# wtsi-svi/ReadServer

Hardware: AMD Instinct MI355X
Metric: 31-mer backward-search queries/sec on popBWT, counted as (query x shard) backward searches/s (higher is better)
Workload: dtype u64

## Files before the change

readserver_amd/csrc/search_solo.h:

```cpp
#ifndef RSBWT_SEARCH_SOLO_H
#define RSBWT_SEARCH_SOLO_H

namespace rsb {

constexpr uint64_t WL_DEAD = 1ull << 63;
constexpr uint32_t SOLO_STAGED_RESULTS = 4u;
constexpr uint32_t SOLO_COUNT_UNSTAGED = 8u;
constexpr uint32_t RES_WAVE_LDS = 2048u;
constexpr uint32_t SOLO_RESULTS_LDS = WG_WAVES * RES_WAVE_LDS;
constexpr uint32_t RES_SLOT_BYTES = 8u;
constexpr uint32_t RES_STATE_BYTES = 8u;
constexpr uint32_t RES_BUFS = RES_WAVE_LDS / (8u * RES_SLOT_BYTES + RES_STATE_BYTES);
static_assert(RES_BUFS * (8u * RES_SLOT_BYTES + RES_STATE_BYTES) <= RES_WAVE_LDS, "a wave's buffers and their state fit its 2 KB");
static_assert(RES_WAVE_LDS == 2048u && RES_BUFS == 28u, "2 KB per wave: with the line slots a CU's 160 KB at four workgroups");
static_assert(RES_BUFS >= 9u && RES_BUFS <= 64u, "a lane per buffer claims; at most 9 groups begin among a pass's 64 draws");
constexpr uint32_t RES_WIDTH_BITS = 24u;
constexpr uint32_t RES_ESCAPED = (1u << RES_WIDTH_BITS) - 1u;

__device__ __forceinline__ void solo_lds_handoff() {
    __builtin_amdgcn_fence(__ATOMIC_RELEASE, "wavefront", "local");
    __builtin_amdgcn_wave_barrier();
    __builtin_amdgcn_fence(__ATOMIC_ACQUIRE, "wavefront", "local");
}

#ifndef RSB_WALK1MM_WGS_PER_CU
#define RSB_WALK1MM_WGS_PER_CU 3
#endif
template <bool COUNT_WORK, bool COUNTS_ONLY, bool LONGK, bool FUSED = false, bool WL = false, bool WALK = false>
__global__ void __launch_bounds__(64 * WG_WAVES, WALK ? RSB_WALK1MM_WGS_PER_CU : RSB_MIN_WGS_PER_CU)
search_solo_kernel(const shard_view *__restrict__ shards, uint32_t nshards, const uint64_t *__restrict__ packed,
                   const ulonglong2 *__restrict__ init, const uint8_t *__restrict__ valid,
                   unsigned long long *__restrict__ next_query,
                   size_t Q, uint32_t k, uint32_t wpq,
                   uint64_t *__restrict__ out_lower, uint64_t *__restrict__ out_upper,
                   unsigned long long *__restrict__ work,
                   ulonglong2 *__restrict__ trace, uint32_t trace_n, uint32_t qchunk, uint32_t pairs_arg,
                   const unsigned long long *__restrict__ wl_counts = nullptr, size_t wl_cap = 0, size_t wl_implicit = 0) {
    __shared__ uint4 s_stage[WG_WAVES][64 * SLOT_U4];
    extern __shared__ uint4 s_results[];
    const uint32_t lane = threadIdx.x & 63u;
    const uint32_t wave = threadIdx.x >> 6;
    uint4 *stage = s_stage[wave];
    const uint32_t stage_lds = __builtin_amdgcn_readfirstlane((uint32_t)(uintptr_t)(lds_void_ptr)stage);
    const uint32_t swz = lane & 7u;
    const uint32_t pairs = pairs_arg & 3u;
    constexpr bool CAN_STAGE = !COUNTS_ONLY && !WL && !WALK;
    const bool stage_out = CAN_STAGE && (pairs_arg & SOLO_STAGED_RESULTS) != 0u && pairs != 2u && Q < (1ull << 34);
    uint2 *results = reinterpret_cast<uint2 *>(s_results + wave * (RES_WAVE_LDS / 16u));
    uint32_t *res_state = reinterpret_cast<uint32_t *>(results + RES_BUFS * 8u);
    const bool count_unstaged = COUNT_WORK && (pairs_arg & SOLO_COUNT_UNSTAGED) != 0u;
    const lds_u32 *mine0 = reinterpret_cast<const lds_u32 *>(stage + (lane & 7u) * 64u + (lane >> 3) * SLOT_U4);
#define SOLO_MINE(d) (mine0 + (((((uint32_t)(d)) >> 2) ^ swz) << 2) + (((uint32_t)(d)) & 3u))

    unsigned long long w_steps = 0, w_occ = 0, w_lines = 0, w_hops = 0, w_ktab = 0, passes = 0;
    unsigned long long w_surv = 0, w_unstepped = 0;
    unsigned long long w_unstaged = 0;

    uint32_t sid = blockIdx.x % nshards;
    for (uint32_t visited = 0; visited < nshards; ++visited, sid = (sid + 1u == nshards) ? 0u : sid + 1u) {
        const shard_view *sv = shards + sid;
        const char *lines_bytes = reinterpret_cast<const char *>(sv->lines);
        const uint32_t S = sv->sp.S;
        const double inv = sv->sp.inv;
        const uint32_t nlines = (uint32_t)sv->nlines;
        const bool ktab = view_uses_ktab(*sv, k);
        const int j_table = ktab ? (int)(k - sv->ktab_depth) - 1 : (int)k - 2;
        const uint32_t w_table = j_table > 0 ? (uint32_t)j_table >> 5 : 0u;
        const ulonglong2 *init_s = WL ? init + (size_t)sid * wl_cap * 2u : init + (size_t)sid * Q;
        const size_t Qs = WALK ? Q : WL ? wl_implicit + (size_t)(wl_counts[(size_t)sid * WL_COUNT_STRIDE] < wl_cap ? wl_counts[(size_t)sid * WL_COUNT_STRIDE] : wl_cap) : Q;
        const uint32_t wl_tn = trace_n, wl_per = WL ? 3u * (k - trace_n) : 1u;
        const size_t walk_V = 3u * (size_t)k + 1u, walk_mv = Q * walk_V;
        ulonglong2 *walk_wl = WALK ? const_cast<ulonglong2 *>(init) + (size_t)sid * wl_cap * 2u : nullptr;
        unsigned long long *walk_count = WALK ? const_cast<unsigned long long *>(wl_counts) + (size_t)sid * WL_COUNT_STRIDE : nullptr;
        uint64_t *out_lo = WALK ? out_lower + (size_t)sid * walk_mv * 2u : out_lower + (size_t)sid * Q * (pairs ? 2u : 1u);
        uint64_t *out_up = (COUNTS_ONLY || pairs) ? nullptr : out_upper + (size_t)sid * Q;
        unsigned long long *pool = next_query + (size_t)sid * POOL_STRIDE;
        if (visited != 0u && __hip_atomic_load(pool, __ATOMIC_RELAXED, __HIP_MEMORY_SCOPE_AGENT) >= (unsigned long long)Qs) continue;
        ulonglong2 *trace_s = (trace && !WL) ? trace + (size_t)sid * Q * trace_n : nullptr;
        const uint64_t *wl_pre = (WL && trace) ? reinterpret_cast<const uint64_t *>(trace) + (size_t)sid * wl_implicit : nullptr;
        unsigned long long *hit_map = pairs == 2u ? reinterpret_cast<unsigned long long *>(out_upper) + (size_t)sid * hit_map_words(WALK ? walk_mv : Q) : nullptr;
        uint32_t ctab_lo, ctab_hi;
        {
            const uint64_t c1 = sv->C[1], c2 = sv->C[2], c3 = sv->C[3], c4 = sv->C[4];
            const uint32_t l3 = lane & 3u;
            const uint64_t cv = l3 == 0u ? c1 : l3 == 1u ? c2 : l3 == 2u ? c3 : c4;
            ctab_lo = (uint32_t)cv;
            ctab_hi = (uint32_t)(cv >> 32);
        }

        const uint64_t *__restrict__ ktab_p = sv->ktab;
        const uint32_t ktab_T = sv->ktab_depth, ktab_stride = sv->ktab_stride, ktab_fmt = sv->ktab_fmt;
        const uint64_t ix_n = sv->n;
        const uint64_t sc1 = sv->C[1], sc2 = sv->C[2], sc3 = sv->C[3], sc4 = sv->C[4];
        const uint64_t st1 = sv->total[1], st2 = sv->total[2], st3 = sv->total[3], st4 = sv->total[4];

        const uint32_t QCHUNK = qchunk;
        if (CAN_STAGE && stage_out && lane < RES_BUFS) {
            res_state[2u * lane] = ~0u;
            res_state[2u * lane + 1u] = 0u;
        }
        uint64_t pool_next = 0, pool_end = 0;
        bool drained = false;
        size_t q = 0;
        bool has_q = false;
        size_t nq = 0;
        bool has_n = false;
        ulonglong2 nrec = {0, 0};
        uint64_t nword = 0;
        uint32_t nstage = 0;
        bool nimp = false;
        int j = 0;
        uint64_t word = 0, lo = 0, hi = 0;
        uint32_t sub = 0;
        uint64_t occL = 0, cacc = 0;
        uint32_t cont = 0, cblk = 0, cdw = 0, co = 0, tries = 0, w = 0;
        uint64_t altL0 = 0, altL1 = 0, altL2 = 0, altU0 = 0, altU1 = 0, altU2 = 0;
        bool alt_ok = true;

        for (;;) {
            bool done = false;
            bool last_in = false;
            if (FUSED && !has_q && has_n && nstage == 2u) {
                const uint64_t e = nrec.x;
                const uint32_t width = (uint32_t)(e >> COUNT_BITS);
                if (nrec.y == 0ull) {
                    nrec.x = INIT_INVALID;
                } else if (width != KTAB_WIDE && (e & COUNT_MASK) + width <= ix_n) {
                    nrec.x = e & COUNT_MASK;
                    nrec.y = nrec.x + width - 1ull;
                } else {
                    const uint32_t bl = (uint32_t)((nword >> (2u * ((k - 1u) & 31u))) & 3u);
                    const uint64_t cb = bl == 0u ? sc1 : bl == 1u ? sc2 : bl == 2u ? sc3 : sc4;
                    const uint64_t tb = bl == 0u ? st1 : bl == 1u ? st2 : bl == 2u ? st3 : st4;
                    nrec.x = cb | INIT_FALLBACK;
                    nrec.y = cb + tb - 1ull;
                }
            }
            if (WL && !has_q && has_n && nstage == 2u) {
                has_q = true;
                has_n = false;
                sub = 0;
                cont = 0;
                word = nword;
                if (nimp) {
                    const uint32_t r_ = (uint32_t)(nrec.y >> 8) & 0xFFu, q_ = (uint32_t)(nrec.y >> 32);
                    const uint32_t pr = (r_ * 171u) >> 9;
                    q = (size_t)q_ * (3u * k + 1u) + 1u + 3u * (wl_tn + pr) + (r_ - 3u * pr);
                    const uint64_t e = nrec.x;
                    const uint32_t width = (uint32_t)(e >> COUNT_BITS);
                    bool tabulated = false;
                    if (width != KTAB_WIDE && (e & COUNT_MASK) + width <= ix_n) {
                        lo = e & COUNT_MASK;
                        hi = lo + width - 1ull;
                        j = (int)wl_tn - 1;
                        tabulated = true;
                    } else {
                        const uint32_t bl = (uint32_t)((nword >> (2u * ((k - 1u) & 31u))) & 3u);
                        const uint64_t cb = bl == 0u ? sc1 : bl == 1u ? sc2 : bl == 2u ? sc3 : sc4;
                        const uint64_t tb = bl == 0u ? st1 : bl == 1u ? st2 : bl == 2u ? st3 : st4;
                        lo = cb;
                        hi = cb + tb - 1ull;
                        j = (int)k - 2;
                    }
                    done = (nrec.y & 0xFFull) == 0ull || (tabulated && lo > hi) || j < 0;
                } else {
                    q = nq;
                    lo = nrec.x & COUNT_MASK;
                    hi = nrec.y;
                    j = (int)((nrec.x >> COUNT_BITS) & 0xFFFFull);
                    done = (nrec.x & WL_DEAD) != 0ull || lo > hi;
                }
                if (done) { lo = 1; hi = 0; }
            }
            if (!WL && !has_q && has_n && (!FUSED || nstage == 2u)) {
                has_q = true;
                has_n = false;
                q = nq;
                sub = 0;
                cont = 0;
                if (nrec.x & INIT_INVALID) {
                    lo = 1;
                    hi = 0;
                    j = -1;
                    done = true;
                } else if (nrec.x & INIT_EXPLICIT) {
                    lo = nrec.x & COUNT_MASK;
                    hi = nrec.y;
                    j = (int)((nrec.x >> COUNT_BITS) & 0xFFFFull) - ((nrec.x & INIT_VAR) ? 1 : 0);
                    word = nword;
                    done = j < 0 || ((nrec.x & INIT_NOCHECK) == 0ull && lo > hi);
                    if (LONGK) {
                        if (!done && ((uint32_t)j >> 5) != w_table) word = packed[q * wpq + ((uint32_t)j >> 5)];
                    }
                } else {
                    const bool fallback = !ktab || (nrec.x & INIT_FALLBACK) != 0ull;
                    lo = nrec.x & COUNT_MASK;
                    hi = nrec.y;
                    j = fallback ? (int)k - 2 : j_table;
                    word = nword;
                    if (COUNT_WORK && !fallback) w_ktab += 1;
                    done = (j < 0) || (!fallback && lo > hi);
                    if (LONGK) {
                        if (!done && ((uint32_t)j >> 5) != w_table) word = packed[q * wpq + ((uint32_t)j >> 5)];
                    }
                }
            }
            if (pool_next >= pool_end && !drained) {
                unsigned long long c = 0;
                if (lane == 0u) c = atomicAdd(pool, (unsigned long long)QCHUNK);
                c = ((unsigned long long)__builtin_amdgcn_readfirstlane((uint32_t)(c >> 32)) << 32) |
                    __builtin_amdgcn_readfirstlane((uint32_t)c);
                pool_next = c;
                pool_end = c + QCHUNK < Qs ? c + QCHUNK : Qs;
                if (c >= Qs) { drained = true; pool_next = pool_end = 0; }
            }
            bool got_n = false;
            {
                const uint64_t want_mask = __builtin_amdgcn_ballot_w64(!has_n);
                const uint32_t before = (uint32_t)__builtin_popcountll(want_mask & ((1ull << lane) - 1ull));
                const uint64_t mine = pool_next + before;
                if (!has_n && mine < pool_end) {
                    nq = (size_t)mine;
                    got_n = true;
                }
                const uint64_t taken = pool_next + (uint32_t)__builtin_popcountll(want_mask);
                const uint64_t r0 = pool_next;
                pool_next = taken < pool_end ? taken : pool_end;
                if (CAN_STAGE && stage_out && pool_next > r0) {
                    const uint64_t first = (r0 + 7ull) & ~7ull;
                    if (first < pool_next) {
                        const uint32_t ga = (uint32_t)(first >> 3), gb = (uint32_t)((pool_next - 1ull) >> 3) + 1u;
                        const uint32_t gam = ga % RES_BUFS;
                        if (lane < RES_BUFS) {
                            const uint32_t d = lane >= gam ? lane - gam : lane + RES_BUFS - gam;
                            const uint32_t g = ga + d;
                            if (g < gb && res_state[2u * lane + 1u] == 0u) {
                                const uint64_t q0 = (uint64_t)g << 3;
                                res_state[2u * lane] = g;
                                res_state[2u * lane + 1u] = (uint32_t)((q0 + 8ull < pool_end ? q0 + 8ull : pool_end) - q0);
                            }
                        }
                    }
                    solo_lds_handoff();
                }
            }
            if (__builtin_amdgcn_ballot_w64(has_q || got_n || ((FUSED || WL) && has_n)) == 0ull) {
                if (drained) break;
                continue;
            }
            ulonglong2 rec = {0, 0};
            uint64_t first_word = 0;
            const bool stage_b = (FUSED || WL) && has_n && nstage == 1u;
            uint64_t entry = 0;
            uint64_t wl_index = 0, vword = 0;
            bool imp = false;
            if (WL) {
                if (got_n) {
                    imp = nq < wl_implicit;
                    if (imp) {
                        const uint32_t i32 = (uint32_t)nq, q_ = i32 / wl_per, r_ = i32 - q_ * wl_per;
                        first_word = packed[q_];
                        rec.y = (uint64_t)valid[q_] | ((uint64_t)r_ << 8) | ((uint64_t)q_ << 32);
                    } else {
                        const size_t slot = nq - wl_implicit;
                        rec = init_s[2u * slot];
                        const ulonglong2 r2 = init_s[2u * slot + 1u];
                        wl_index = r2.x;
                        first_word = r2.y;
                    }
                }
                if (stage_b) {
                    const uint32_t r_ = (uint32_t)(nrec.y >> 8) & 0xFFu;
                    const uint32_t pr = (r_ * 171u) >> 9, d_ = r_ - 3u * pr, p_ = wl_tn + pr;
                    const uint32_t orig = (uint32_t)((nword >> (2u * p_)) & 3u);
                    const uint32_t alt = d_ < orig ? d_ : d_ + 1u;
                    vword = nword ^ ((uint64_t)(orig ^ alt) << (2u * p_));
                    const uint64_t code = (vword >> (2u * wl_tn)) & ((1ull << (2u * ktab_T)) - 1ull);
                    entry = wl_pre ? wl_pre[nq] : ktab_entry(ktab_p, ktab_fmt, ktab_T, ktab_stride, code);
                }
            } else if (FUSED) {
                if (got_n) {
                    rec.y = valid[nq];
                    first_word = packed[nq];
                }
                if (stage_b) {
                    const uint64_t code = (nword >> (2u * (k - ktab_T))) & ((1ull << (2u * ktab_T)) - 1ull);
                    entry = ktab_entry(ktab_p, ktab_fmt, ktab_T, ktab_stride, code);
                }
            } else if (got_n) {
                rec = init_s[nq];
                first_word = packed[nq * wpq + w_table];
            }
            const bool alive = has_q;
            const bool stepping = alive && !done;
            const bool fresh = stepping && cont == 0u;

            uint32_t b = 1, line = 0, o = 0;
            if (stepping) {
                if (LONGK) {
                    if (fresh && sub == 0u && (j & 31) == 31) word = packed[q * wpq + ((uint32_t)j >> 5)];
                }
                b = (uint32_t)((word >> (2u * ((uint32_t)j & 31u))) & 3u) + 1u;
            }
            bool no_fetch = false;
            if (fresh) {
                if (sub == 0u) {
                    if (WALK) {
                        alt_ok = true;
                        altL0 = altL1 = altL2 = altU0 = altU1 = altU2 = 0;
                    }
                    if (trace_s && (uint32_t)j < trace_n) trace_s[q * trace_n + (uint32_t)j] = make_ulonglong2(lo, hi);
                    if (lo == 0ull) {
                        occL = 0;
                        sub = 1u;
                    }
                }
                const uint64_t p = sub ? hi : lo - 1ull;
                if (p == ~0ull) {
                    no_fetch = true;
                } else {
                    uint32_t pin;
                    w = fast_window(p, S, inv, pin);
                    line = w + (w >> GROUP_SHIFT);
                    o = pin + 1u;
                    if (line >= nlines) line = 0;
                    if (COUNT_WORK) w_occ += 1;
                }
            }
            const bool looking = stepping && !no_fetch;
            const uint64_t pb = ((uint64_t)(uint32_t)__builtin_amdgcn_ds_bpermute((int)((b - 1u) << 2), (int)ctab_hi) << 32) |
                                (uint32_t)__builtin_amdgcn_ds_bpermute((int)((b - 1u) << 2), (int)ctab_lo);

            const uint32_t want = looking ? (cont ? cblk : line) : ~0u;
            if (COUNT_WORK && want != ~0u) {
                if (cont) w_hops += 1;
                else w_lines += 1;
            }
            glds_fetch(lines_bytes, want, lane, stage_lds);
            glds_wait();

            bool do_scan = false, own_line = false;
            uint64_t base = 0, cnt_b = 0;
            uint32_t dw = HDR_DWORDS, rem = 0, oe_here = 0;
            uint32_t s1 = 0, s2 = 0, s3 = 0, span = 0, hb = 0;
            const sym_tab stab = make_sym_tab(b);
            if (looking) {
                if (cont != KIND_CHUNK) {
                    const uint32_t oe = cont ? co : o;
                    const uint2 cw = *reinterpret_cast<const lds_u2 *>(SOLO_MINE(2u * (b - 1u)));
                    const uint4 h0 = *reinterpret_cast<const lds_u4 *>(SOLO_MINE(0));
                    const uint64_t cnt = ((uint64_t)(cw.y & 0xFFu) << 32) | cw.x;
                    const uint32_t m0 = h0.y >> 8, m1 = h0.w >> 8;
                    s1 = m0 & 0x3FFu;
                    s2 = (m0 >> 10) & 0x7FFu;
                    s3 = s2 + (m1 & 0x3FFu);
                    span = s3 + ((m1 >> 10) & 0x3FFu);
                    const uint32_t kind = (m1 >> 20) & 3u;
                    if (oe <= span) {
                        const uint32_t cq = (oe > s1 ? 1u : 0u) + (oe > s2 ? 1u : 0u) + (oe > s3 ? 1u : 0u);
                        const uint32_t start = cq == 0u ? 0u : cq == 1u ? s1 : cq == 2u ? s2 : s3;
                        const uint32_t hm = *SOLO_MINE(5u + 2u * ((b - 1u) >> 1)) >> 8;
                        hb = (hm >> (11u * ((b - 1u) & 1u))) & 0x7FFu;
                        const uint32_t qd = HDR_DWORDS + 6u * (cq & 2u);
                        const uint2 x0 = *reinterpret_cast<const lds_u2 *>(SOLO_MINE(qd));
                        const uint2 x1 = *reinterpret_cast<const lds_u2 *>(SOLO_MINE(qd + 2u));
                        const uint2 x2 = *reinterpret_cast<const lds_u2 *>(SOLO_MINE(qd + 4u));
                        const uint32_t e6[6] = {x0.x, x0.y, x1.x, x1.y, x2.x, x2.y};
                        const uint32_t m = matched24_tab(e6, stab);
                        base = cnt + (cq >= 2u ? hb : 0u) + ((cq & 1u) ? m : 0u);
                        dw = HDR_DWORDS + 6u * cq;
                        rem = oe - start;
                        do_scan = true;
                        own_line = true;
                        oe_here = oe;
                        cnt_b = cnt;
                    } else if (kind == KIND_FAR) {
                        cblk = *SOLO_MINE(LINE_DWORDS - 1u);
                        if (cblk >= nlines) cblk = 0;
                        cont = KIND_FAR;
                        co = oe - span;
                    } else if (kind == KIND_CHUNK && cont == 0u) {
                        const uint32_t m2 = *SOLO_MINE(5) >> 8, m3 = *SOLO_MINE(7) >> 8;
                        cacc = cnt;
                        cdw = 2u * (((m2 >> 22) & 3u) | (((m3 >> 22) & 3u) << 2));
                        cblk = (w >> GROUP_SHIFT) * (GROUP + 1u) + GROUP;
                        if (cblk >= nlines) cblk = 0;
                        cont = KIND_CHUNK;
                        co = oe - span;
                    } else {
                        base = cnt;
                        do_scan = true;
                    }
                } else {
                    const uint2 hd = *reinterpret_cast<const lds_u2 *>(SOLO_MINE(cdw));
                    const uint32_t hw = (b <= 2u) ? hd.x : hd.y;
                    const uint32_t tot = (hw >> (12u * ((b - 1u) & 1u))) & 0xFFFu;
                    base = cacc + tot;
                    dw = cdw + 2u;
                    rem = co;
                    do_scan = true;
                }
                if (!do_scan && ++tries > 72u) do_scan = true;
            }
            uint64_t occ = 0;
            {
                const uint2 y0 = *reinterpret_cast<const lds_u2 *>(SOLO_MINE(dw & 31u));
                const uint2 y1 = *reinterpret_cast<const lds_u2 *>(SOLO_MINE((dw + 2u) & 31u));
                const uint2 y2 = *reinterpret_cast<const lds_u2 *>(SOLO_MINE((dw + 4u) & 31u));
                const uint32_t r6[6] = {y0.x, y0.y, y1.x, y1.y, y2.x, y2.y};
                occ = base + rank24(r6, stab, b, rem);
#ifdef RSB_FAULT_INJECT_WILD_OCC
                if ((((uint32_t)q + (uint32_t)j) * 2654435761u >> 28) == 0u)
                    occ = (occ + (((uint64_t)q * 0x9E3779B97F4A7C15ull) >> (23u + (((uint32_t)q + (uint32_t)j) & 31u)))) & ((1ull << 41) - 1ull);
#endif
            }
            bool step_done = false;
            uint64_t occU = 0;
            bool second = false;
            uint32_t oh = 0;
            bool ev1 = false, ev1_is_L = false;
            if (WALK && do_scan && (uint32_t)j < trace_n) {
                if (own_line) {
                    ev1 = true;
                    ev1_is_L = sub == 0u;
                } else {
                    alt_ok = false;
                }
            }
            if (do_scan) {
                cont = 0;
                tries = 0;
                if (sub == 0u) {
                    occL = occ;
                    sub = 1u;
                    const uint64_t d = hi - (lo - 1ull);
                    if (own_line && d <= (uint64_t)(span - oe_here)) {
                        second = true;
                        oh = oe_here + (uint32_t)d;
                    }
                } else {
                    occU = occ;
                    step_done = true;
                }
            }
            {
                const uint32_t cq = (oh > s1 ? 1u : 0u) + (oh > s2 ? 1u : 0u) + (oh > s3 ? 1u : 0u);
                const uint32_t start = cq == 0u ? 0u : cq == 1u ? s1 : cq == 2u ? s2 : s3;
                const uint32_t qd = HDR_DWORDS + 6u * (cq & 2u);
                const uint2 x0 = *reinterpret_cast<const lds_u2 *>(SOLO_MINE(qd));
                const uint2 x1 = *reinterpret_cast<const lds_u2 *>(SOLO_MINE(qd + 2u));
                const uint2 x2 = *reinterpret_cast<const lds_u2 *>(SOLO_MINE(qd + 4u));
                const uint32_t e6[6] = {x0.x, x0.y, x1.x, x1.y, x2.x, x2.y};
                const uint32_t m = matched24_tab(e6, stab);
                const uint32_t dw2 = HDR_DWORDS + 6u * cq;
                const uint2 y0 = *reinterpret_cast<const lds_u2 *>(SOLO_MINE(dw2));
                const uint2 y1 = *reinterpret_cast<const lds_u2 *>(SOLO_MINE(dw2 + 2u));
                const uint2 y2 = *reinterpret_cast<const lds_u2 *>(SOLO_MINE(dw2 + 4u));
                const uint32_t r6[6] = {y0.x, y0.y, y1.x, y1.y, y2.x, y2.y};
                const uint32_t sc = rank24(r6, stab, b, second ? oh - start : 0u);
                if (second) {
                    occU = cnt_b + (cq >= 2u ? hb : 0u) + ((cq & 1u) ? m : 0u) + sc;
                    step_done = true;
                    if (COUNT_WORK) w_occ += 1;
                }
            }
            if (stepping && no_fetch) {
                occU = 0;
                step_done = true;
            }
            if (WALK) {
                const staged_line Lrow = {mine0, swz};
                const line_head hh = {s1, s2, s3, span, 0u};
#pragma unroll 1
                for (uint32_t ev = 0; ev < 2u; ++ev) {
                    const bool want = ev == 0u ? ev1 : (second && (uint32_t)j < trace_n);
                    if (__builtin_amdgcn_ballot_w64(want) == 0ull) continue;
                    uint64_t t3[3];
                    staged_occ_alts(Lrow, hh, want ? (ev == 0u ? oe_here : oh) : 1u, b - 1u, t3);
                    if (want) {
                        if (ev == 0u && ev1_is_L) { altL0 = t3[0]; altL1 = t3[1]; altL2 = t3[2]; }
                        else { altU0 = t3[0]; altU1 = t3[1]; altU2 = t3[2]; }
                    }
                }
                const bool emit = step_done && (uint32_t)j < trace_n;
                if (__builtin_amdgcn_ballot_w64(emit) != 0ull) {
                    const uint32_t orig = b - 1u;
                    uint64_t nlo[3], nhi[3], masks[3];
                    bool enq[3];
#pragma unroll
                    for (uint32_t d = 0; d < 3u; ++d) {
                        const uint32_t alt = d < orig ? d : d + 1u;
                        const uint64_t cb = ((uint64_t)(uint32_t)__builtin_amdgcn_ds_bpermute((int)(alt << 2), (int)ctab_hi) << 32) |
                                            (uint32_t)__builtin_amdgcn_ds_bpermute((int)(alt << 2), (int)ctab_lo);
                        nlo[d] = cb + (d == 0u ? altL0 : d == 1u ? altL1 : altL2);
                        nhi[d] = cb + (d == 0u ? altU0 : d == 1u ? altU1 : altU2) - 1ull;
                        const bool stepped_live = emit && alt_ok && nlo[d] <= nhi[d];
                        const bool final_hit = stepped_live && j == 0;
                        enq[d] = (stepped_live && j != 0) || (emit && !alt_ok);
                        if (final_hit) {
                            const size_t canon = q * walk_V + 1u + 3u * (uint32_t)j + d;
                            reinterpret_cast<ulonglong2 *>(out_lo)[canon] = make_ulonglong2(nlo[d], nhi[d]);
                            atomicOr(hit_map + (canon >> 6), 1ull << (canon & 63u));
                        }
                        masks[d] = __builtin_amdgcn_ballot_w64(enq[d]);
                        if (COUNT_WORK) {
                            w_surv += __builtin_popcountll(__builtin_amdgcn_ballot_w64((enq[d] && alt_ok) || final_hit));
                            w_unstepped += __builtin_popcountll(__builtin_amdgcn_ballot_w64(enq[d] && !alt_ok));
                        }
                    }
                    if (COUNT_WORK && emit) w_steps += 3;
                    const uint32_t n0 = (uint32_t)__builtin_popcountll(masks[0]), n1 = (uint32_t)__builtin_popcountll(masks[1]);
                    const uint32_t total = n0 + n1 + (uint32_t)__builtin_popcountll(masks[2]);
                    if (total != 0u) {
                        unsigned long long wbase = 0;
                        if (lane == 0u) wbase = atomicAdd(walk_count, (unsigned long long)total);
                        wbase = ((unsigned long long)(uint32_t)__builtin_amdgcn_readfirstlane((int)(uint32_t)(wbase >> 32)) << 32) |
                                (uint32_t)__builtin_amdgcn_readfirstlane((int)(uint32_t)wbase);
                        const uint64_t lt = (1ull << lane) - 1ull;
#pragma unroll
                        for (uint32_t d = 0; d < 3u; ++d) {
                            if (!enq[d]) continue;
                            const size_t slot = (size_t)wbase + (d >= 1u ? n0 : 0u) + (d >= 2u ? n1 : 0u) + (size_t)__builtin_popcountll(masks[d] & lt);
                            if (slot >= wl_cap) continue;
                            const uint32_t alt = d < orig ? d : d + 1u;
                            const uint64_t vword = word ^ ((uint64_t)(orig ^ alt) << (2u * (uint32_t)j));
                            const uint64_t canon = (uint64_t)q * walk_V + 1ull + 3ull * (uint32_t)j + d;
                            if (!alt_ok) wl_store(walk_wl, slot, lo, (uint32_t)j, hi, canon, vword);
                            else wl_store(walk_wl, slot, nlo[d], (uint32_t)j - 1u, nhi[d], canon, vword);
                        }
                    }
                }
            }
            if (step_done) {
                if (COUNT_WORK) w_steps += 1;
                lo = pb + occL;
                hi = pb + occU - 1ull;
                --j;
                done = (lo > hi) || (j < 0);
                sub = 0;
            }
            if ((FUSED || WL) && stage_b) {
                nrec.x = entry;
                nstage = 2u;
                if (WL) nword = vword;
            }
            if (got_n) {
                nrec = rec;
                nword = first_word;
                has_n = true;
                nstage = (WL && !imp) ? 2u : 1u;
                nimp = imp;
                if (WL && !imp) nq = (size_t)wl_index;
            }
            if (CAN_STAGE && stage_out) solo_lds_handoff();
            if (alive && done) {
                if (trace_s) {
                    for (int jj = j < (int)trace_n ? j : (int)trace_n - 1; jj >= 0; --jj)
                        trace_s[q * trace_n + (uint32_t)jj] = make_ulonglong2(lo, hi);
                }
                if (COUNTS_ONLY) {
                    if (hi >= lo) out_lo[q] = hi - lo + 1ull;
                } else if (pairs == 2u) {
                    if (lo <= hi) {
                        const size_t qi = WALK ? q * walk_V : q;
                        reinterpret_cast<ulonglong2 *>(out_lo)[qi] = make_ulonglong2(lo, hi);
                        atomicOr(hit_map + (qi >> 6), 1ull << (qi & 63u));
                    }
                } else {
                    const uint32_t g32 = (uint32_t)(q >> 3), rb = g32 % RES_BUFS;
                    bool own_store = true;
                    if (CAN_STAGE && stage_out && res_state[2u * rb] == g32) {
                        const uint64_t width = hi - lo + 1ull;
                        own_store = width >= (uint64_t)RES_ESCAPED || (lo >> COUNT_BITS) != 0ull;
                        results[rb * 8u + ((uint32_t)q & 7u)] =
                            own_store ? make_uint2(0u, RES_ESCAPED << 8) : make_uint2((uint32_t)lo, (uint32_t)(lo >> 32) | ((uint32_t)width << 8));
                        last_in = atomicSub(&res_state[2u * rb + 1u], 1u) == 1u;
                    }
                    if (own_store) {
                        if (pairs) {
                            reinterpret_cast<ulonglong2 *>(out_lo)[q] = make_ulonglong2(lo, hi);
                        } else {
                            out_lo[q] = lo;
                            out_up[q] = hi;
                        }
                        if (count_unstaged) w_unstaged += 1;
                    }
                }
                has_q = false;
            }
            if (CAN_STAGE && stage_out) {
                solo_lds_handoff();
                uint64_t fm = __builtin_amdgcn_ballot_w64(last_in);
                while (fm != 0ull) {
                    const int src = __builtin_ctzll(fm);
                    fm &= fm - 1ull;
                    const uint32_t g = (uint32_t)__builtin_amdgcn_readlane((int)(uint32_t)(q >> 3), src), bsel = g % RES_BUFS;
                    const size_t qq = ((size_t)g << 3) + lane;
                    if (lane < 8u && qq < Qs) {
                        const uint2 v = results[bsel * 8u + lane];
                        const uint32_t width = v.y >> 8;
                        const uint64_t vlo = ((uint64_t)(v.y & 0xFFu) << 32) | v.x, vhi = vlo + width - 1ull;
                        if (width == RES_ESCAPED) {
                        } else if (pairs) {
                            reinterpret_cast<ulonglong2 *>(out_lo)[qq] = make_ulonglong2(vlo, vhi);
                        } else {
                            out_lo[qq] = vlo;
                            out_up[qq] = vhi;
                        }
                    }
                }
            }
            if (COUNT_WORK) ++passes;
        }
    }
    if (COUNT_WORK) {
        if (lane == 0u) atomicAdd(&work[WORK_PASSES], passes);
        if (threadIdx.x == 0u && blockIdx.x == 0u) work[WORK_SOLO] = 1ull;
        if (w_steps) atomicAdd(&work[WORK_STEPS], w_steps);
        if (w_occ) atomicAdd(&work[WORK_OCC], w_occ);
        if (w_lines) atomicAdd(&work[WORK_LINES], w_lines);
        if (w_ktab) atomicAdd(&work[WORK_KTAB], w_ktab);
        if (w_hops) atomicAdd(&work[WORK_HOPS], w_hops);
        if (w_unstaged) atomicAdd(&work[WORK_UNSTAGED], w_unstaged);
        if (WALK && lane == 0u) {
            atomicAdd(&work[13], w_surv);
            atomicAdd(&work[14], w_unstepped);
        }
    }
#undef SOLO_MINE
}

}
#endif
```

Before: 4.247 billion.

## Reuse lower-bound window fetch for upper bound when both fall in same window

When computing the lower occurrence, the code now records whether the upper bound lies in the same sampling window. If so, it reuses the already-fetched line for the upper rank. That covers the first chunk of a FAR/CHUNK continuation, or a second rank inside the staged chunk. This is meant to skip a separate line fetch and hop chain for the upper bound. In exchange it adds state tracking (a flag bit packed into the `tries` field), extra branches and register pressure, and a risk of wrong continuation offsets.

Result: faster. 4.336 billion, median of 6 (+2.1%).

```diff
diff --git a/readserver_amd/csrc/search_solo.h b/readserver_amd/csrc/search_solo.h
--- a/readserver_amd/csrc/search_solo.h
+++ b/readserver_amd/csrc/search_solo.h
@@ -114,6 +114,7 @@
         uint32_t sub = 0;
         uint64_t occL = 0, cacc = 0;
         uint32_t cont = 0, cblk = 0, cdw = 0, co = 0, tries = 0, w = 0;
+        constexpr uint32_t SAME_WINDOW = 1u << 31;
         uint64_t altL0 = 0, altL1 = 0, altL2 = 0, altU0 = 0, altU1 = 0, altU2 = 0;
         bool alt_ok = true;
 
@@ -325,6 +326,7 @@
                     o = pin + 1u;
                     if (line >= nlines) line = 0;
                     if (COUNT_WORK) w_occ += 1;
+                    if (sub == 0u) tries = hi - p <= (uint64_t)(S - o) ? SAME_WINDOW : 0u;
                 }
             }
             const bool looking = stepping && !no_fetch;
@@ -340,13 +342,16 @@
             glds_wait();
 
             bool do_scan = false, own_line = false;
-            uint64_t base = 0, cnt_b = 0;
-            uint32_t dw = HDR_DWORDS, rem = 0, oe_here = 0;
+            uint64_t base = 0;
+            uint32_t dw = HDR_DWORDS, rem = 0;
             uint32_t s1 = 0, s2 = 0, s3 = 0, span = 0, hb = 0;
             const sym_tab stab = make_sym_tab(b);
+            const uint32_t cont_in = cont;
+            uint32_t more = 0;
             if (looking) {
                 if (cont != KIND_CHUNK) {
-                    const uint32_t oe = cont ? co : o;
+                    if (cont == 0u) co = o;
+                    const uint32_t oe = co;
                     const uint2 cw = *reinterpret_cast<const lds_u2 *>(SOLO_MINE(2u * (b - 1u)));
                     const uint4 h0 = *reinterpret_cast<const lds_u4 *>(SOLO_MINE(0));
                     const uint64_t cnt = ((uint64_t)(cw.y & 0xFFu) << 32) | cw.x;
@@ -356,6 +361,18 @@
                     s3 = s2 + (m1 & 0x3FFu);
                     span = s3 + ((m1 >> 10) & 0x3FFu);
                     const uint32_t kind = (m1 >> 20) & 3u;
+                    cacc = cnt;
+                    if (kind == KIND_FAR) {
+                        cblk = *SOLO_MINE(LINE_DWORDS - 1u);
+                        if (cblk >= nlines) cblk = 0;
+                        more = KIND_FAR;
+                    } else if (kind == KIND_CHUNK && cont == 0u) {
+                        const uint32_t m2 = *SOLO_MINE(5) >> 8, m3 = *SOLO_MINE(7) >> 8;
+                        cdw = 2u * (((m2 >> 22) & 3u) | (((m3 >> 22) & 3u) << 2));
+                        cblk = (w >> GROUP_SHIFT) * (GROUP + 1u) + GROUP;
+                        if (cblk >= nlines) cblk = 0;
+                        more = KIND_CHUNK;
+                    }
                     if (oe <= span) {
                         const uint32_t cq = (oe > s1 ? 1u : 0u) + (oe > s2 ? 1u : 0u) + (oe > s3 ? 1u : 0u);
                         const uint32_t start = cq == 0u ? 0u : cq == 1u ? s1 : cq == 2u ? s2 : s3;
@@ -372,20 +389,8 @@
                         rem = oe - start;
                         do_scan = true;
                         own_line = true;
-                        oe_here = oe;
-                        cnt_b = cnt;
-                    } else if (kind == KIND_FAR) {
-                        cblk = *SOLO_MINE(LINE_DWORDS - 1u);
-                        if (cblk >= nlines) cblk = 0;
-                        cont = KIND_FAR;
-                        co = oe - span;
-                    } else if (kind == KIND_CHUNK && cont == 0u) {
-                        const uint32_t m2 = *SOLO_MINE(5) >> 8, m3 = *SOLO_MINE(7) >> 8;
-                        cacc = cnt;
-                        cdw = 2u * (((m2 >> 22) & 3u) | (((m3 >> 22) & 3u) << 2));
-                        cblk = (w >> GROUP_SHIFT) * (GROUP + 1u) + GROUP;
-                        if (cblk >= nlines) cblk = 0;
-                        cont = KIND_CHUNK;
+                    } else if (more != 0u) {
+                        cont = more;
                         co = oe - span;
                     } else {
                         base = cnt;
@@ -400,7 +405,7 @@
                     rem = co;
                     do_scan = true;
                 }
-                if (!do_scan && ++tries > 72u) do_scan = true;
+                if (!do_scan && (++tries & ~SAME_WINDOW) > 72u) do_scan = true;
             }
             uint64_t occ = 0;
             {
@@ -416,9 +421,10 @@
             }
             bool step_done = false;
             uint64_t occU = 0;
-            bool second = false;
+            bool second = false, second_chunk = false;
             uint32_t oh = 0;
             bool ev1 = false, ev1_is_L = false;
+            const uint32_t co_in = co;
             if (WALK && do_scan && (uint32_t)j < trace_n) {
                 if (own_line) {
                     ev1 = true;
@@ -428,15 +434,23 @@
                 }
             }
             if (do_scan) {
+                const bool same_w = (tries & SAME_WINDOW) != 0u;
                 cont = 0;
                 tries = 0;
                 if (sub == 0u) {
                     occL = occ;
                     sub = 1u;
                     const uint64_t d = hi - (lo - 1ull);
-                    if (own_line && d <= (uint64_t)(span - oe_here)) {
+                    if (own_line && d <= (uint64_t)(span - co)) {
                         second = true;
-                        oh = oe_here + (uint32_t)d;
+                        oh = co + (uint32_t)d;
+                    } else if (own_line && same_w && more != 0u) {
+                        cont = more;
+                        co = co + (uint32_t)d - span;
+                        if (COUNT_WORK) w_occ += 1;
+                    } else if (cont_in == KIND_CHUNK && same_w) {
+                        second_chunk = true;
+                        oh = co + (uint32_t)d;
                     }
                 } else {
                     occU = occ;
@@ -452,14 +466,14 @@
                 const uint2 x2 = *reinterpret_cast<const lds_u2 *>(SOLO_MINE(qd + 4u));
                 const uint32_t e6[6] = {x0.x, x0.y, x1.x, x1.y, x2.x, x2.y};
                 const uint32_t m = matched24_tab(e6, stab);
-                const uint32_t dw2 = HDR_DWORDS + 6u * cq;
-                const uint2 y0 = *reinterpret_cast<const lds_u2 *>(SOLO_MINE(dw2));
-                const uint2 y1 = *reinterpret_cast<const lds_u2 *>(SOLO_MINE(dw2 + 2u));
-                const uint2 y2 = *reinterpret_cast<const lds_u2 *>(SOLO_MINE(dw2 + 4u));
+                const uint32_t dw2 = second_chunk ? dw : HDR_DWORDS + 6u * cq;
+                const uint2 y0 = *reinterpret_cast<const lds_u2 *>(SOLO_MINE(dw2 & 31u));
+                const uint2 y1 = *reinterpret_cast<const lds_u2 *>(SOLO_MINE((dw2 + 2u) & 31u));
+                const uint2 y2 = *reinterpret_cast<const lds_u2 *>(SOLO_MINE((dw2 + 4u) & 31u));
                 const uint32_t r6[6] = {y0.x, y0.y, y1.x, y1.y, y2.x, y2.y};
-                const uint32_t sc = rank24(r6, stab, b, second ? oh - start : 0u);
-                if (second) {
-                    occU = cnt_b + (cq >= 2u ? hb : 0u) + ((cq & 1u) ? m : 0u) + sc;
+                const uint32_t sc = rank24(r6, stab, b, second ? oh - start : second_chunk ? oh : 0u);
+                if (second || second_chunk) {
+                    occU = second ? cacc + (cq >= 2u ? hb : 0u) + ((cq & 1u) ? m : 0u) + sc : base + sc;
                     step_done = true;
                     if (COUNT_WORK) w_occ += 1;
                 }
@@ -476,7 +490,7 @@
                     const bool want = ev == 0u ? ev1 : (second && (uint32_t)j < trace_n);
                     if (__builtin_amdgcn_ballot_w64(want) == 0ull) continue;
                     uint64_t t3[3];
-                    staged_occ_alts(Lrow, hh, want ? (ev == 0u ? oe_here : oh) : 1u, b - 1u, t3);
+                    staged_occ_alts(Lrow, hh, want ? (ev == 0u ? co_in : oh) : 1u, b - 1u, t3);
                     if (want) {
                         if (ev == 0u && ev1_is_L) { altL0 = t3[0]; altL1 = t3[1]; altL2 = t3[2]; }
                         else { altU0 = t3[0]; altU1 = t3[1]; altU2 = t3[2]; }
```
